# Daaohame/RAHT-3DGS-codec

Measured on AMD Instinct MI355X. Metric: M-Gaussians/s fwd+inv RAHT, 59-ch SH3 3DGS, higher is better.
Workload: dtype f32 (xyz columns: f64); 1 GPU; cfg3: 2999072 Gaussians (3000000 draws/GPU, J=12, 59 channels), fwd RAHT + quantize/reorder + dequantize/un-reorder + inv RAHT (quantization fused into the transform kernels); the 3 xyz columns carried in float64 inside the same launches (raht_fwd_quant_mixed / raht_dequant_inv_mixed): the reference's integers on every column; rows_per_gpu=2999072, channels=59, depth_J=12, engine=tile, quantize=True, parallelism=1 GPU, world=1

## Files before the change

raht-3dgs-codec_amd/csrc/raht_device.h:

```cpp
#pragma once
#include "raht_common.h"

namespace raht {

struct StepTable {
    int n;
    int fast_div;
    float v[MAX_STEP_CH];
};
struct NoSteps { int n; int fast_div; };
struct StepTable64 { int n; double v[MAX_STEP_CH]; };
template <typename T> struct StepsFor;
template <> struct StepsFor<float> { typedef StepTable type; typedef float elem; };
template <> struct StepsFor<double> { typedef StepTable64 type; typedef double elem; };


template <typename E> struct alignas(16) RegChunk { E v[16 / sizeof(E)]; };
template <typename E> struct __attribute__((packed, aligned(sizeof(E)))) MemChunk { E v[16 / sizeof(E)]; };

template <typename E, bool STREAM = false>
__device__ __forceinline__ RegChunk<E> ld_chunk(const E *__restrict__ p)
{
    constexpr int VN = 16 / sizeof(E);
    RegChunk<E> x;
    if constexpr (STREAM) {
#pragma unroll
        for (int i = 0; i < VN; ++i) x.v[i] = __builtin_nontemporal_load(p + i);
    } else {
        const MemChunk<E> t = *(const MemChunk<E> *)p;
#pragma unroll
        for (int i = 0; i < VN; ++i) x.v[i] = t.v[i];
    }
    return x;
}

template <typename E, bool STREAM = false>
__device__ __forceinline__ void st_chunk(E *__restrict__ p, const RegChunk<E> &x)
{
    constexpr int VN = 16 / sizeof(E);
    if constexpr (STREAM) {
#pragma unroll
        for (int i = 0; i < VN; ++i) __builtin_nontemporal_store(x.v[i], p + i);
    } else {
        MemChunk<E> t;
#pragma unroll
        for (int i = 0; i < VN; ++i) t.v[i] = x.v[i];
        *(MemChunk<E> *)p = t;
    }
}

template <int VN> struct __attribute__((packed, aligned(4))) IntPack { int32_t v[VN]; };
// ... 142 lines not shown
```

raht-3dgs-codec_amd/csrc/transform.hip:

```cpp
#include "raht_common.h"
#include "raht_device.h"
#include "tile_engine.h"
#include "tile_host.h"

#include <algorithm>
#include <type_traits>
#include <vector>

namespace raht {

size_t tile_lds_bytes(int R, int elem_size, int Dc, bool ident, bool qm);

template <typename T> struct Vec16;
template <> struct Vec16<float> { typedef float4 type; static constexpr int n = 4; };
template <> struct Vec16<double> { typedef double2 type; static constexpr int n = 2; };

template <typename T>
__global__ void copy_rows_kernel(const T *__restrict__ src, int64_t lds, T *__restrict__ dst, int64_t ldd,
                                 int64_t N, int D)
{
    const int64_t total = N * D;
    for (int64_t e = (int64_t)blockIdx.x * blockDim.x + threadIdx.x; e < total;
         e += (int64_t)gridDim.x * blockDim.x) {
        const int64_t i = e / D;
// ... 642 lines not shown
template <typename T, bool INV, bool IDENT, bool QM, int SLOTS>
__global__ __launch_bounds__(TILE_THREADS, (sizeof(T) == 4 ? 6 : 4)) void tile_kernel_batch(const TileBatch<T> B,
                                                   const typename std::conditional<QM, typename StepsFor<T>::type, NoSteps>::type ST)
{
    int s = 0;
#pragma unroll
    for (int q = 1; q < BATCH_MAX; ++q) s += (q < B.n && blockIdx.x >= B.first_tile[q]) ? 1 : 0;
    const int64_t t = (int64_t)(blockIdx.x - B.first_tile[s]);
    tile_body<T, INV, IDENT, QM, SLOTS>(B.a[s], ST, t, (int64_t)1 << 40, (int)blockIdx.y);
}

constexpr int TOP_THREADS = 1024;
constexpr int TOP_SLOTS = RAHT_TOP_MAX_ROWS / TOP_THREADS;

template <typename T>
struct TopArgs {
    const T *in;  int64_t ld_in;
    T *fin;       int64_t ld_fin;
    T *out;       int64_t ld_out;
    int32_t *Q;   int64_t ldq;
    const uint32_t *rows;
    int io_mapped;
    const uint32_t *e_pos;
    const uint32_t *pj;
    const T *ab;
    const uint32_t *root_rank;
    T *root_buf;
    int n, n_merges, D;
    const uint32_t *lev;
    int nlev, nbig;
    uint32_t small_start;
};

template <typename T, bool INV, bool QM, bool MULTI = false>
__device__ __forceinline__ void top_body(const TopArgs<T> &A, const typename std::conditional<QM, typename StepsFor<T>::type, NoSteps>::type &ST,
                                         const int chunk, const MultiQ *MQ = nullptr)
{
    constexpr bool QM64 = QM && sizeof(T) == 8;
    extern __shared__ __align__(16) unsigned char smem[];
    typedef RegChunk<T> V16;
    constexpr int VN = 16 / sizeof(T);
    V16 *tile = (V16 *)smem;
    __shared__ uint32_t s_lev[2 * 64];
    const int tid = threadIdx.x;
    const int goff = min(chunk * VN, A.D - VN);
    const int n = A.n, nm = A.n_merges;
    if (tid < 2 * A.nlev) s_lev[tid] = A.lev[tid];
    const int n_small = nm - (int)A.small_start;
    uint32_t *s_pj = (uint32_t *)(smem + (size_t)n * 16);
    T *s_ab = (T *)(s_pj + ((n_small + 3) & ~3));
    for (int i = tid; i < n_small; i += TOP_THREADS) {
        s_pj[i] = A.pj[A.small_start + i];
        s_ab[2 * i] = A.ab[2 * (A.small_start + i)];
        s_ab[2 * i + 1] = A.ab[2 * (A.small_start + i) + 1];
    }

    typename StepsFor<T>::elem my_step[VN];
    float my_rcp[VN];
#pragma unroll
    for (int i = 0; i < VN; ++i) { my_step[i] = 1; my_rcp[i] = 1.0f; }
    if constexpr (QM) {
#pragma unroll
        for (int i = 0; i < VN; ++i) {
            my_step[i] = ST.v[ST.n == 1 ? 0 : goff + i];
            if constexpr (!QM64) my_rcp[i] = refined_rcp(my_step[i]);
        }
    }

    uint32_t pj[TOP_SLOTS];
    T ra[TOP_SLOTS], rb[TOP_SLOTS];
#pragma unroll
    for (int k = 0; k < TOP_SLOTS; ++k) {
        const int idx = min(k * TOP_THREADS + tid, max(nm - 1, 0));
        pj[k] = A.pj[idx]; ra[k] = A.ab[2 * idx]; rb[k] = A.ab[2 * idx + 1];
    }
    uint32_t m_dst[TOP_SLOTS], m_rr[TOP_SLOTS];
#pragma unroll
    for (int k = 0; k < TOP_SLOTS; ++k) {
        const int e = min(k * TOP_THREADS + tid, n - 1);
        m_rr[k] = A.root_rank[e];
        m_dst[k] = QM ? A.e_pos[e] : (A.rows ? A.rows[e] : (uint32_t)e);
    }
    {
        typedef typename std::conditional<QM && INV && !QM64, int32_t, T>::type RawT;
        RegChunk<RawT> x[TOP_SLOTS];
#pragma unroll
        for (int k = 0; k < TOP_SLOTS; ++k) {
            const int e = min(k * TOP_THREADS + tid, n - 1);
            if constexpr (QM64 && INV) {
                int32_t q[VN];
                ld_ints<VN>(A.Q + (int64_t)m_dst[k] * A.ldq + goff, q);
#pragma unroll
                for (int i = 0; i < VN; ++i) x[k].v[i] = (T)q[i];
            } else if constexpr (!INV) {
                x[k] = ld_chunk<RawT>((const RawT *)A.in + (int64_t)(A.io_mapped ? m_dst[k] : (uint32_t)e) * A.ld_in + goff);
            } else if constexpr (QM) {
                x[k] = ld_chunk<RawT>((const RawT *)A.Q + (int64_t)m_dst[k] * A.ldq + goff);
            } else {
                const T *src = (A.root_buf && m_rr[k] != 0xffffffffu) ? A.root_buf + (int64_t)m_rr[k] * A.D
                                                                      : A.fin + (int64_t)m_dst[k] * A.ld_fin;
                x[k] = ld_chunk<RawT>((const RawT *)src + goff);
            }
        }
#pragma unroll
        for (int k = 0; k < TOP_SLOTS; ++k) {
            const int e = k * TOP_THREADS + tid;
            if (e < n) {
                V16 v;
#pragma unroll
                for (int i = 0; i < VN; ++i) {
                    v.v[i] = (T)x[k].v[i];
                    if constexpr (QM && INV) v.v[i] = v.v[i] * (T)my_step[i];
                }
                tile[e] = v;
            }
        }
        if constexpr (QM && INV) {
            if (A.root_buf) {
#pragma unroll
                for (int k = 0; k < TOP_SLOTS; ++k) {
                    const int e = k * TOP_THREADS + tid;
                    if (e < n && m_rr[k] != 0xffffffffu) tile[e] = ld_chunk<T>(A.root_buf + (int64_t)m_rr[k] * A.D + goff);
                }
            }
        }
    }
    __syncthreads();

    auto butterfly = [&](uint32_t rec, T a, T b) {
        const uint32_t ip = rec & 0xffffu, ij = rec >> 16;
        const V16 x0 = tile[ip], x1 = tile[ij];
        V16 vlo, vhi;
#pragma unroll
        for (int i = 0; i < VN; ++i) {
            if (!INV) {
                vlo.v[i] = a * x0.v[i] + b * x1.v[i];
                vhi.v[i] = a * x1.v[i] - b * x0.v[i];
            } else {
                vlo.v[i] = a * x0.v[i] - b * x1.v[i];
                vhi.v[i] = b * x0.v[i] + a * x1.v[i];
            }
        }
        tile[ip] = vlo; tile[ij] = vhi;
    };
    auto big_levels = [&]() {
#pragma unroll 1
        for (int q = 0; q < A.nbig; ++q) {
            const int li = INV ? A.nbig - 1 - q : q;
            const uint32_t lo = s_lev[2 * li], hi = s_lev[2 * li + 1];
#pragma unroll
            for (int k = 0; k < TOP_SLOTS; ++k) {
                const uint32_t idx = (uint32_t)(k * TOP_THREADS + tid);
                if ((uint32_t)(k * TOP_THREADS) < hi && (uint32_t)((k + 1) * TOP_THREADS) > lo && idx >= lo && idx < hi)
                    butterfly(pj[k], ra[k], rb[k]);
            }
            __syncthreads();
        }
    };
    auto small_levels = [&]() {
        if (tid < 64) {
#pragma unroll 1
            for (int q = A.nbig; q < A.nlev; ++q) {
                const int li = INV ? A.nlev - 1 - (q - A.nbig) : q;
                const uint32_t lo = s_lev[2 * li], hi = s_lev[2 * li + 1];
                const uint32_t i = lo - A.small_start + (uint32_t)tid;
                if (lo + (uint32_t)tid < hi) butterfly(s_pj[i], s_ab[2 * i], s_ab[2 * i + 1]);
            }
        }
        __syncthreads();
    };
    if (!INV) { big_levels(); small_levels(); }
    else { small_levels(); big_levels(); }

#pragma unroll
    for (int k = 0; k < TOP_SLOTS; ++k) {
        const int e = k * TOP_THREADS + tid;
        if (e >= n) continue;
        const V16 v = tile[e];
        if constexpr (INV) {
            st_chunk<T>(A.out + (int64_t)(A.io_mapped ? m_dst[k] : (uint32_t)e) * A.ld_out + goff, v);
        } else {
            const uint32_t rr = m_rr[k];
            const bool to_buf = A.root_buf && rr != 0xffffffffu;
            if (to_buf) st_chunk<T>(A.root_buf + (int64_t)rr * A.D + goff, v);
            if (QM && to_buf) {
            } else if constexpr (QM) {
                if constexpr (QM64) {
                    int32_t qv[VN];
#pragma unroll
                    for (int i = 0; i < VN; ++i) qv[i] = quantize_one_f64((double)v.v[i], (double)my_step[i]);
                    st_ints<VN>(A.Q + (int64_t)m_dst[k] * A.ldq + goff, qv);
                } else if constexpr (MULTI) {
                    for (int kk = 0; kk < MQ->k; ++kk) {
                        const float sp = MQ->step[kk], rc = refined_rcp(sp);
                        RegChunk<int32_t> qv;
#pragma unroll
                        for (int i = 0; i < VN; ++i) qv.v[i] = quantize_one((float)v.v[i], sp, rc, MQ->fast_div);
                        st_chunk<int32_t>(MQ->Q[kk] + (int64_t)m_dst[k] * A.ldq + goff, qv);
                    }
                } else {
                    RegChunk<int32_t> qv;
#pragma unroll
                    for (int i = 0; i < VN; ++i) qv.v[i] = quantize_one((float)v.v[i], (float)my_step[i], my_rcp[i], ST.fast_div);
                    st_chunk<int32_t>(A.Q + (int64_t)m_dst[k] * A.ldq + goff, qv);
                }
            } else {
                st_chunk<T>(A.fin + (int64_t)m_dst[k] * A.ld_fin + goff, v);
            }
        }
    }
}

template <typename T, bool INV, bool QM>
__global__ __launch_bounds__(TOP_THREADS) void top_kernel(const TopArgs<T> A,
                                                          const typename std::conditional<QM, typename StepsFor<T>::type, NoSteps>::type ST)
{
    top_body<T, INV, QM>(A, ST, (int)blockIdx.x);
}

__global__ __launch_bounds__(TOP_THREADS) void top_kernel_multi(const TopArgs<float> A, const StepTable ST, const MultiQ M)
{
    top_body<float, false, true, true>(A, ST, (int)blockIdx.x, &M);
}

template <typename T>
struct TopBatch { TopArgs<T> a[BATCH_MAX]; };

template <typename T, bool INV, bool QM>
__global__ __launch_bounds__(TOP_THREADS) void top_kernel_batch(const TopBatch<T> B,
                                                                const typename std::conditional<QM, typename StepsFor<T>::type, NoSteps>::type ST)
{
    top_body<T, INV, QM>(B.a[blockIdx.y], ST, (int)blockIdx.x);
}

template <typename T>
__global__ void node_weight_kernel(const int32_t *__restrict__ wl, const int32_t *__restrict__ wr,
                                   const int64_t *__restrict__ wsum, int64_t N, T *__restrict__ w)
{
    const int64_t i = (int64_t)blockIdx.x * blockDim.x + threadIdx.x;
    if (i >= N) return;
    if (i == 0) { w[0] = (T)(wsum ? wsum[N] : N); return; }
    double w0, w1;
    pair_weights(i, wl[i], wr[i], wsum, w0, w1);
    w[i] = (T)(w0 + w1);
}

static int lp_shift_for(int Dc)
{
    int s = 0;
    while ((1 << s) < Dc && s < 6) ++s;
// ... 119 lines not shown
        else if (st.tile_rows < 1 || (int64_t)st.tile_rows * std::max<int64_t>(std::max(A.ld_in, A.ld_out), A.ld_fin) * (int64_t)sizeof(T) >= ((int64_t)1 << 32)) bad = "tile geometry (32-bit row offsets)";
        if (bad) { set_error("tile stage %d (%s): missing %s", k, INV ? "inverse" : "forward", bad); return RAHT_ERR_INVALID; }
    }
    G.nchunks = (unsigned)((D + Dc - 1) / Dc);
    G.lds = tile_lds_bytes(st.tile_rows, (int)sizeof(T), Dc, st.rows == nullptr, QM);
    if (st.tile_rows > TILE_MAX_SLOTS * TILE_THREADS) {
        set_error("tile_rows %d too large for %d threads", st.tile_rows, TILE_THREADS);
        return RAHT_ERR_UNSUPPORTED;
    }
    G.n_tiles = st.n_tiles;
    G.one = st.tile_rows <= TILE_THREADS;
    G.ident = st.rows == nullptr;
    if (sq) {
        if (G.nchunks != 1 || !G.ident || (size_t)(TILE_THREADS / 64) * (size_t)(((D + 3) / 4) * 4) * 8 > G.lds) {
            set_error("raht_dequant_inv_sqdiff: unexpected stage-0 geometry");
            return RAHT_ERR_INVALID;
        }
        if (!A.out) A.ld_out = 0;
        A.ref = io.ref; A.ld_ref = io.ld_ref; A.sq_part = io.sq_part;
    }
    return RAHT_OK;
}

template <typename T, bool INV, bool QM>
static int launch_prepared(const raht_plan *p, int k, const StageLaunch<T> &L, const XformIO<T> &io, bool events, hipStream_t s)
{
    constexpr bool F32Q = QM && std::is_same<T, float>::value;
    const auto st = steps_arg<T, QM>(io);
    auto launch = [&]() -> int {
        if (L.is_top) {
            constexpr int VN = 16 / (int)sizeof(T);
            const dim3 grid((unsigned)((L.P.D + VN - 1) / VN)), block(TOP_THREADS);
            if constexpr (F32Q && !INV) { if (io.multi) return launch_lds<top_kernel_multi>(grid, block, L.G.lds, TOP_LDS_LIMIT, s, L.P, st, *io.multi); }
            return launch_lds<top_kernel<T, INV, QM>>(grid, block, L.G.lds, TOP_LDS_LIMIT, s, L.P, st);
        }
        const TileGeom &G = L.G;
        const dim3 grid((unsigned)G.n_tiles, G.nchunks), block(TILE_THREADS);
        return by_ident_slots(G.ident, G.one, [&](auto ident, auto slots) -> int {
            constexpr bool IDENT = decltype(ident)::value;
            constexpr int SLOTS = decltype(slots)::value;
            if constexpr (F32Q && !INV) { if (io.multi) return launch_lds<tile_kernel_multi<IDENT, SLOTS>>(grid, block, G.lds, TILE_LDS_LIMIT, s, L.A, st, *io.multi); }
            if constexpr (F32Q && INV && IDENT) { if (L.A.sq_part) return launch_lds<tile_kernel_sq<SLOTS>>(grid, block, G.lds, TILE_LDS_LIMIT, s, L.A, st); }
            return launch_lds<tile_kernel<T, INV, IDENT, QM, SLOTS>>(grid, block, G.lds, TILE_LDS_LIMIT, s, L.A, st);
        });
    };
    if (!(events && k == 0 && p->ev_before)) return launch();
    RAHT_HIP_CHECK(hipEventRecord(p->ev_before, s));
    const int rc = launch();
    RAHT_HIP_CHECK(hipEventRecord(p->ev_after, s));
    return rc;
}

template <typename T, bool INV, bool QM>
static int launch_stage(const raht_plan *p, const Schedule &sc, int k, const XformIO<T> &io, int D, int Dc0, hipStream_t s, int dbg = 0)
{
    StageLaunch<T> L;
    RAHT_RET((prepare_stage<T, INV, QM>(p, sc, k, io, D, Dc0, dbg, L)));
    return launch_prepared<T, INV, QM>(p, k, L, io, dbg == 0, s);
}

template <typename T, bool INV, bool QM>
static int launch_tile_batch(int m, const StageLaunch<T> *const *Ls, const XformIO<T> &io, hipStream_t s)
{
    TileBatch<T> B;
    B.n = m;
    uint32_t tot = 0;
    for (int i = 0; i < BATCH_MAX; ++i) {
// ... 490 lines not shown
```

raht-3dgs-codec_amd/csrc/transform_mx.hip:

```cpp
#include "raht_common.h"
#include "raht_device.h"
#include "tile_engine.h"
#include "tile_host.h"

#include <algorithm>
#include <cstdlib>
#include <string>
#include <type_traits>
#include <vector>

namespace raht {

#ifdef RAHT_PHASE_CLOCKS
constexpr int MX_CLK_TILES = 4096, MX_CLK_SLOTS = 12;
__device__ unsigned long long g_phase_clk_mx[MX_CLK_TILES][MX_CLK_SLOTS];
#define MX_STAMP(k) do { if (IDENT && threadIdx.x == 0 && tile_id < MX_CLK_TILES) g_phase_clk_mx[tile_id][k] = __builtin_readcyclecounter(); } while (0)
#else
#define MX_STAMP(k) do { } while (0)
#endif

constexpr int MX_MAX_WIDE = 4;
constexpr int MX_THREADS = 512;
constexpr int MX_TOP_THREADS = 1024;
constexpr int MX_TOP_SLOTS = RAHT_TOP_MAX_ROWS / MX_TOP_THREADS;
// ... 586 lines not shown
    TileArgs<float> a[BATCH_MAX];
    MxPtrs p[BATCH_MAX];
    uint32_t first_tile[BATCH_MAX + 1];
    int n;
};
static_assert(sizeof(TileBatchMX) + sizeof(StepTableMX) <= 4096, "tile_kernel_mx_batch: arguments exceed the 4 KB kernarg segment");

template <bool INV, bool IDENT, int SLOTS>
__global__ __launch_bounds__(MX_THREADS, 6) void tile_kernel_mx_batch(const TileBatchMX B, const StepTableMX ST)
{
    int s = 0;
#pragma unroll
    for (int q = 1; q < BATCH_MAX; ++q) s += (q < B.n && blockIdx.x >= B.first_tile[q]) ? 1 : 0;
    tile_body_mx<INV, IDENT, SLOTS, false>(B.a[s], B.p[s], ST, (int64_t)(blockIdx.x - B.first_tile[s]));
}

struct TopArgsMX {
    const float *in_rows;  int64_t ld_in;
    const float *in_img; const double *in_img_w;
    float *out_rows;       int64_t ld_out;
    float *out_img; double *out_img_w;
    int32_t *Q;            int64_t ldq;
    const uint32_t *e_pos;
    const uint32_t *pj;
    const float *ab32;  const double *ab64;
    int n, n_merges, D, nwide, Fp;
    const uint32_t *lev;
    int nlev, nbig;
    uint32_t small_start;
    const uint32_t *root_rank;
    float *root_f; double *root_w;
};

template <bool WIDE, bool INV, bool ROOTS, bool MULTI = false>
__device__ __forceinline__ void top_body_mx(const TopArgsMX &A, const StepTableMX &ST, const int chunk, const MxMultiQ *MQ = nullptr)
{
    typedef typename std::conditional<WIDE, double, float>::type T;
    constexpr int VN = WIDE ? 2 : 4;
    typedef RegChunk<T> V16;
    extern __shared__ __align__(16) unsigned char smem[];
    V16 *tile = (V16 *)smem;
    __shared__ uint32_t s_lev[2 * 64];
    const int tid = threadIdx.x;
    const int nwide = A.nwide;
    const int goff = WIDE ? 2 * chunk : min(chunk * 4, A.D - 4);
    const int ioff = chunk * 4;
    const int n = A.n, nm = A.n_merges;
    if (tid < 2 * A.nlev) s_lev[tid] = A.lev[tid];
    const T *ab = WIDE ? (const T *)A.ab64 : (const T *)A.ab32;
    const int n_small = nm - (int)A.small_start;
    uint32_t *s_pj = (uint32_t *)(smem + (size_t)n * 16);
    T *s_ab = (T *)(s_pj + ((n_small + 3) & ~3));
    for (int i = tid; i < n_small; i += MX_TOP_THREADS) {
        s_pj[i] = A.pj[A.small_start + i];
        s_ab[2 * i] = ab[2 * (A.small_start + i)];
        s_ab[2 * i + 1] = ab[2 * (A.small_start + i) + 1];
    }
    T my_step[VN];
    float my_rcp[VN];
    bool live[VN];
#pragma unroll
    for (int i = 0; i < VN; ++i) {
        if constexpr (WIDE) { live[i] = goff + i < nwide; my_step[i] = live[i] ? ST.w[goff + i] : 1.0; my_rcp[i] = 1.0f; }
        else { live[i] = !(chunk == 0 && i < nwide); my_step[i] = ST.f.v[ST.f.n == 1 ? 0 : goff + i]; my_rcp[i] = refined_rcp(my_step[i]); }
    }
    uint32_t pj[MX_TOP_SLOTS];
    T ra[MX_TOP_SLOTS], rb[MX_TOP_SLOTS];
#pragma unroll
    for (int k = 0; k < MX_TOP_SLOTS; ++k) {
        const int idx = min(k * MX_TOP_THREADS + tid, max(nm - 1, 0));
        pj[k] = A.pj[idx]; ra[k] = ab[2 * idx]; rb[k] = ab[2 * idx + 1];
    }
    uint32_t m_dst[MX_TOP_SLOTS], m_rr[MX_TOP_SLOTS];
#pragma unroll
    for (int k = 0; k < MX_TOP_SLOTS; ++k) {
        m_dst[k] = A.e_pos[min(k * MX_TOP_THREADS + tid, n - 1)];
        m_rr[k] = ROOTS ? A.root_rank[min(k * MX_TOP_THREADS + tid, n - 1)] : 0xffffffffu;
    }
#pragma unroll
    for (int k = 0; k < MX_TOP_SLOTS; ++k) {
        const int e = k * MX_TOP_THREADS + tid;
        if (e >= n) continue;
        V16 v;
        if constexpr (!INV) {
            if (A.in_img) {
                if constexpr (WIDE) {
#pragma unroll
                    for (int i = 0; i < VN; ++i) v.v[i] = live[i] ? A.in_img_w[(int64_t)e * nwide + goff + i] : 0.0;
                } else {
                    v = *(const V16 *)(A.in_img + (int64_t)e * A.Fp + ioff);
                }
            } else if constexpr (WIDE) {
#pragma unroll
                for (int i = 0; i < VN; ++i) v.v[i] = live[i] ? (double)A.in_rows[(int64_t)e * A.ld_in + goff + i] : 0.0;
            } else {
                v = ld_chunk<float>(A.in_rows + (int64_t)e * A.ld_in + goff);
            }
        } else if (m_rr[k] != 0xffffffffu) {
            if constexpr (WIDE) {
#pragma unroll
                for (int i = 0; i < VN; ++i) v.v[i] = live[i] ? A.root_w[(int64_t)m_rr[k] * nwide + goff + i] : 0.0;
            } else {
                v = ld_chunk<float>(A.root_f + (int64_t)m_rr[k] * A.D + goff);
            }
        } else {
            const int32_t *q = A.Q + (int64_t)m_dst[k] * A.ldq + goff;
            if constexpr (WIDE) {
#pragma unroll
                for (int i = 0; i < VN; ++i) v.v[i] = live[i] ? (double)q[i] * my_step[i] : 0.0;
            } else {
                const RegChunk<int32_t> raw = ld_chunk<int32_t>(q);
#pragma unroll
                for (int i = 0; i < VN; ++i) v.v[i] = (float)raw.v[i] * my_step[i];
            }
        }
        tile[e] = v;
    }
    __syncthreads();

    auto butterfly = [&](uint32_t rec, T a, T b) {
        const uint32_t ip = rec & 0xffffu, ij = rec >> 16;
        const V16 x0 = tile[ip], x1 = tile[ij];
        V16 vlo, vhi;
#pragma unroll
        for (int i = 0; i < VN; ++i) {
            if (!INV) {
                vlo.v[i] = a * x0.v[i] + b * x1.v[i];
                vhi.v[i] = a * x1.v[i] - b * x0.v[i];
            } else {
                vlo.v[i] = a * x0.v[i] - b * x1.v[i];
                vhi.v[i] = b * x0.v[i] + a * x1.v[i];
            }
        }
        tile[ip] = vlo; tile[ij] = vhi;
    };
    auto big_levels = [&]() {
#pragma unroll 1
        for (int q = 0; q < A.nbig; ++q) {
            const int li = INV ? A.nbig - 1 - q : q;
            const uint32_t lo = s_lev[2 * li], hi = s_lev[2 * li + 1];
#pragma unroll
            for (int k = 0; k < MX_TOP_SLOTS; ++k) {
                const uint32_t idx = (uint32_t)(k * MX_TOP_THREADS + tid);
                if ((uint32_t)(k * MX_TOP_THREADS) < hi && (uint32_t)((k + 1) * MX_TOP_THREADS) > lo && idx >= lo && idx < hi)
                    butterfly(pj[k], ra[k], rb[k]);
            }
            __syncthreads();
        }
    };
    auto small_levels = [&]() {
        if (tid < 64) {
#pragma unroll 1
            for (int q = A.nbig; q < A.nlev; ++q) {
                const int li = INV ? A.nlev - 1 - (q - A.nbig) : q;
                const uint32_t lo = s_lev[2 * li], hi = s_lev[2 * li + 1];
                const uint32_t i = lo - A.small_start + (uint32_t)tid;
                if (lo + (uint32_t)tid < hi) butterfly(s_pj[i], s_ab[2 * i], s_ab[2 * i + 1]);
            }
        }
        __syncthreads();
    };
    if (!INV) { big_levels(); small_levels(); }
    else { small_levels(); big_levels(); }

#pragma unroll
    for (int k = 0; k < MX_TOP_SLOTS; ++k) {
        const int e = k * MX_TOP_THREADS + tid;
        if (e >= n) continue;
        const V16 v = tile[e];
        if constexpr (INV) {
            if (A.out_img) {
                if constexpr (WIDE) {
#pragma unroll
                    for (int i = 0; i < VN; ++i) if (live[i]) A.out_img_w[(int64_t)e * nwide + goff + i] = v.v[i];
                } else {
                    *(V16 *)(A.out_img + (int64_t)e * A.Fp + ioff) = v;
                }
            } else if constexpr (WIDE) {
#pragma unroll
                for (int i = 0; i < VN; ++i) if (live[i]) A.out_rows[(int64_t)e * A.ld_out + goff + i] = (float)v.v[i];
            } else if (chunk == 0) {
#pragma unroll
                for (int i = 0; i < VN; ++i) if (live[i]) A.out_rows[(int64_t)e * A.ld_out + goff + i] = v.v[i];
            } else {
                st_chunk<float>(A.out_rows + (int64_t)e * A.ld_out + goff, v);
            }
        } else if (m_rr[k] != 0xffffffffu) {
            if constexpr (WIDE) {
#pragma unroll
                for (int i = 0; i < VN; ++i) if (live[i]) A.root_w[(int64_t)m_rr[k] * nwide + goff + i] = v.v[i];
            } else {
                st_chunk<float>(A.root_f + (int64_t)m_rr[k] * A.D + goff, v);
            }
        } else if constexpr (MULTI) {
            for (int kk = 0; kk < MQ->k; ++kk) {
                int32_t *q = MQ->Q[kk] + (int64_t)m_dst[k] * A.ldq + goff;
                if constexpr (WIDE) {
#pragma unroll
                    for (int i = 0; i < VN; ++i) if (live[i]) q[i] = quantize_one_f64(v.v[i], MQ->step[kk]);
                } else {
                    const float sf = (float)MQ->step[kk], rf = refined_rcp(sf);
                    const int fd = (int)((MQ->fast_div >> kk) & 1u);
                    RegChunk<int32_t> qv;
#pragma unroll
                    for (int i = 0; i < VN; ++i) qv.v[i] = quantize_one(v.v[i], sf, rf, fd);
                    if (chunk == 0) {
#pragma unroll
                        for (int i = 0; i < VN; ++i) if (live[i]) q[i] = qv.v[i];
                    } else {
                        st_chunk<int32_t>(q, qv);
                    }
                }
            }
        } else {
            int32_t *q = A.Q + (int64_t)m_dst[k] * A.ldq + goff;
            if constexpr (WIDE) {
#pragma unroll
                for (int i = 0; i < VN; ++i) if (live[i]) q[i] = quantize_one_f64(v.v[i], my_step[i]);
            } else {
                RegChunk<int32_t> qv;
#pragma unroll
                for (int i = 0; i < VN; ++i) qv.v[i] = quantize_one(v.v[i], my_step[i], my_rcp[i], ST.f.fast_div);
                if (chunk == 0) {
#pragma unroll
                    for (int i = 0; i < VN; ++i) if (live[i]) q[i] = qv.v[i];
                } else {
                    st_chunk<int32_t>(q, qv);
                }
            }
        }
    }
}

template <bool INV>
__global__ __launch_bounds__(MX_TOP_THREADS) void top_kernel_mx(const TopArgsMX A, const StepTableMX ST)
{
    const int NW2 = (A.nwide + 1) >> 1;
    if ((int)blockIdx.x < NW2) top_body_mx<true, INV, false>(A, ST, (int)blockIdx.x);
    else top_body_mx<false, INV, false>(A, ST, (int)blockIdx.x - NW2);
}
template <bool INV>
__global__ __launch_bounds__(MX_TOP_THREADS) void top_kernel_mx_roots(const TopArgsMX A, const StepTableMX ST)
{
    const int NW2 = (A.nwide + 1) >> 1;
    if ((int)blockIdx.x < NW2) top_body_mx<true, INV, true>(A, ST, (int)blockIdx.x);
    else top_body_mx<false, INV, true>(A, ST, (int)blockIdx.x - NW2);
}

struct TopBatchMX { TopArgsMX a[BATCH_MAX]; };
static_assert(sizeof(TopBatchMX) + sizeof(StepTableMX) <= 4096, "top_kernel_mx_batch: arguments exceed the 4 KB kernarg segment");

template <bool INV>
__global__ __launch_bounds__(MX_TOP_THREADS) void top_kernel_mx_batch(const TopBatchMX B, const StepTableMX ST)
{
    const TopArgsMX &A = B.a[blockIdx.y];
    const int NW2 = (A.nwide + 1) >> 1;
    if ((int)blockIdx.x < NW2) top_body_mx<true, INV, false>(A, ST, (int)blockIdx.x);
    else top_body_mx<false, INV, false>(A, ST, (int)blockIdx.x - NW2);
}

__global__ __launch_bounds__(MX_TOP_THREADS) void top_kernel_mx_multi(const TopArgsMX A, const StepTableMX ST, const MxMultiQ M)
{
    const int NW2 = (A.nwide + 1) >> 1;
    if ((int)blockIdx.x < NW2) top_body_mx<true, false, false, true>(A, ST, (int)blockIdx.x, &M);
    else top_body_mx<false, false, false, true>(A, ST, (int)blockIdx.x - NW2, &M);
}

__global__ void mx_cols_to_f64_kernel(const float *__restrict__ C, int64_t ldc, int64_t N, int nwide, double *__restrict__ W)
{
    const int64_t e = (int64_t)blockIdx.x * blockDim.x + threadIdx.x;
    if (e >= N * nwide) return;
    const int64_t i = e / nwide;
// ... 140 lines not shown
        else if (INV && !A.out && !(k == 0 && io.sq_part)) bad = "inverse output";
        else if (k == 0 && io.sq_part && (!INV || !io.ref || A.root_buf || (int64_t)st.tile_rows * io.ld_ref * 4 >= ((int64_t)1 << 31))) bad = "sqdiff reference rows";
        else if (!INV && io.multi && A.root_buf) bad = "multi-step write-back without root buffers";
        else if ((st.rows == nullptr) != (k == 0)) bad = "stage order";
        else if (st.tile_rows < 1 || st.tile_rows > TILE_MAX_SLOTS * MX_THREADS ||
                 (int64_t)st.tile_rows * std::max<int64_t>(io.ldc, g.Dp) * 4 >= ((int64_t)1 << 31)) bad = "tile geometry (32-bit row offsets)";
        if (bad) { set_error("mixed tile stage %d (%s): missing %s", k, INV ? "inverse" : "forward", bad); return RAHT_ERR_INVALID; }
    }
    MxPtrs &P = L.P;
    P.in_w = (!INV && k >= 1) ? ws_k_w : nullptr;
    P.out_w = (INV && k >= 1) ? ws_k_w : nullptr;
    P.wsn_w = ws_n_w;
    P.root_w = A.last_stage ? p->root_buf_w : nullptr;
    P.prog = st.prog; P.prog_stride = st.prog_stride; P.prog_ab = st.prog_ab; P.prog_compact = st.prog_compact ? 1 : 0;
    if (!P.prog) { set_error("mixed tile stage %d: missing tile programs", k); return RAHT_ERR_INVALID; }
    L.lds = tile_lds_bytes_mx(st.tile_rows, g.Dp / 4, g.nwide);
    L.n_tiles = (unsigned)st.n_tiles;
    if (INV && k == 0 && io.sq_part) {
        A.out = io.C_out; A.ld_out = io.C_out ? io.ldc : 0;
        A.ref = io.ref; A.ld_ref = io.ld_ref; A.sq_part = io.sq_part;
    }
    return RAHT_OK;
}

template <bool INV>
static int launch_prepared_mx(const raht_plan *p, int k, const MxIO &io, const MxStageLaunch &L, const MxGeom &g,
                              const StepTableMX &stp, hipStream_t s)
{
    auto launch = [&]() -> int {
        if (L.is_top) {
            const dim3 grid((unsigned)g.NCp), block(MX_TOP_THREADS);
            if constexpr (!INV) { if (io.multi) return launch_lds<top_kernel_mx_multi>(grid, block, L.lds, TOP_LDS_LIMIT, s, L.T, stp, *io.multi); }
            if (L.T.root_f) return launch_lds<top_kernel_mx_roots<INV>>(grid, block, L.lds, TOP_LDS_LIMIT, s, L.T, stp);
            return launch_lds<top_kernel_mx<INV>>(grid, block, L.lds, TOP_LDS_LIMIT, s, L.T, stp);
        }
        if constexpr (!INV) { if (io.multi) return launch_tile_mx<false, false, MX_MULTI>(k == 0, L.A, L.P, stp, io.multi, L.n_tiles, L.lds, s); }
        if constexpr (INV) { if (k == 0 && io.sq_part) return launch_tile_mx<true, false, MX_SQ>(true, L.A, L.P, stp, nullptr, L.n_tiles, L.lds, s); }
        return L.A.root_buf ? launch_tile_mx<INV, true, MX_PLAIN>(k == 0, L.A, L.P, stp, nullptr, L.n_tiles, L.lds, s)
                            : launch_tile_mx<INV, false, MX_PLAIN>(k == 0, L.A, L.P, stp, nullptr, L.n_tiles, L.lds, s);
    };
    if (!(k == 0 && p->ev_before)) return launch();
    RAHT_HIP_CHECK(hipEventRecord(p->ev_before, s));
    const int rc = launch();
    RAHT_HIP_CHECK(hipEventRecord(p->ev_after, s));
    return rc;
}

template <bool INV>
static int launch_stage_mx(const raht_plan *p, const Schedule &sc, int k, const MxIO &io, int D, const MxGeom &g,
                           const StepTableMX &stp, hipStream_t s)
{
    MxStageLaunch L;
    RAHT_RET((prepare_stage_mx<INV>(p, sc, k, io, D, g, L)));
    return launch_prepared_mx<INV>(p, k, io, L, g, stp, s);
}

static int mx_check_args(const raht_plan *p, const void *a, const void *b, int D, int64_t lda, int64_t ldb, const double *steps,
                         int n_steps, int n_wide, const char *what)
{
    if (!p || !a || !b || D < 1 || lda < D || ldb < D) { set_error("%s: bad argument", what); return RAHT_ERR_INVALID; }
    RAHT_RET(check_plan_device(p, what));
    if (n_wide < 1 || n_wide > MX_MAX_WIDE || n_wide > D) { set_error("%s: n_wide must be 1..%d (and <= D)", what, MX_MAX_WIDE); return RAHT_ERR_INVALID; }
    RAHT_RET(check_quant_steps(what, steps, n_steps, D, true));
    if (p->row_map) { set_error("%s: not available for row-mapped plans", what); return RAHT_ERR_UNSUPPORTED; }
    if ((p->root_buf == nullptr) != (p->root_buf_w == nullptr)) {
        set_error("%s: set both root buffers (raht_plan_set_root_buffer and raht_plan_set_root_buffer_wide) or neither", what);
        return RAHT_ERR_UNSUPPORTED;
// ... 433 lines not shown
```

Baseline: 5001 M-Gaussians/s.

## Restructure top-level RAHT kernel loads for latency hiding and specialize slot count

The top-of-tree kernels now issue index, row-chunk and root loads up front, batched between scheduling barriers, and stage the small-level merge records into LDS through registers after the main loads are issued. Slot count becomes a template parameter, so small top levels launch with 1 or 2 slots and skip unused loads and butterflies. The store loop exits per wave rather than per lane. The aim is to cut serialized global-memory latency in these small, latency-bound top kernels, at the cost of more registers and extra kernel instantiations.

```diff
diff --git a/raht-3dgs-codec_amd/csrc/raht_device.h b/raht-3dgs-codec_amd/csrc/raht_device.h
--- a/raht-3dgs-codec_amd/csrc/raht_device.h
+++ b/raht-3dgs-codec_amd/csrc/raht_device.h
@@ -17,6 +17,7 @@
 
 template <typename E> struct alignas(16) RegChunk { E v[16 / sizeof(E)]; };
 template <typename E> struct __attribute__((packed, aligned(sizeof(E)))) MemChunk { E v[16 / sizeof(E)]; };
+struct __attribute__((packed, aligned(4), may_alias)) RawChunk { uint32_t v[4]; };
 
 template <typename E, bool STREAM = false>
 __device__ __forceinline__ RegChunk<E> ld_chunk(const E *__restrict__ p)
diff --git a/raht-3dgs-codec_amd/csrc/transform.hip b/raht-3dgs-codec_amd/csrc/transform.hip
--- a/raht-3dgs-codec_amd/csrc/transform.hip
+++ b/raht-3dgs-codec_amd/csrc/transform.hip
@@ -698,7 +698,7 @@
     uint32_t small_start;
 };
 
-template <typename T, bool INV, bool QM, bool MULTI = false>
+template <typename T, bool INV, bool QM, bool MULTI = false, int SLOTS = TOP_SLOTS>
 __device__ __forceinline__ void top_body(const TopArgs<T> &A, const typename std::conditional<QM, typename StepsFor<T>::type, NoSteps>::type &ST,
                                          const int chunk, const MultiQ *MQ = nullptr)
 {
@@ -711,15 +711,36 @@
     const int tid = threadIdx.x;
     const int goff = min(chunk * VN, A.D - VN);
     const int n = A.n, nm = A.n_merges;
-    if (tid < 2 * A.nlev) s_lev[tid] = A.lev[tid];
+    uint32_t m_dst[SLOTS], m_rr[SLOTS];
+#pragma unroll
+    for (int k = 0; k < SLOTS; ++k) {
+        const int e = min(k * TOP_THREADS + tid, n - 1);
+        m_rr[k] = A.root_rank[e];
+        m_dst[k] = QM ? A.e_pos[e] : (A.rows ? A.rows[e] : (uint32_t)e);
+    }
+    const uint32_t lev_word = A.lev[min(tid, 2 * 64 - 1)];
     const int n_small = nm - (int)A.small_start;
     uint32_t *s_pj = (uint32_t *)(smem + (size_t)n * 16);
     T *s_ab = (T *)(s_pj + ((n_small + 3) & ~3));
-    for (int i = tid; i < n_small; i += TOP_THREADS) {
-        s_pj[i] = A.pj[A.small_start + i];
-        s_ab[2 * i] = A.ab[2 * (A.small_start + i)];
-        s_ab[2 * i + 1] = A.ab[2 * (A.small_start + i) + 1];
-    }
+    constexpr int STAGE = 2;
+    const int nm_last = max(nm - 1, 0);
+    uint32_t g_pj[STAGE];
+    T g_a[STAGE], g_b[STAGE];
+    auto stage_load = [&](int base) {
+#pragma unroll
+        for (int q = 0; q < STAGE; ++q) {
+            const int idx = min((int)A.small_start + base + q * TOP_THREADS + tid, nm_last);
+            g_pj[q] = A.pj[idx]; g_a[q] = A.ab[2 * idx]; g_b[q] = A.ab[2 * idx + 1];
+        }
+    };
+    auto stage_store = [&](int base) {
+#pragma unroll
+        for (int q = 0; q < STAGE; ++q) {
+            const int i = base + q * TOP_THREADS + tid;
+            if (i < n_small) { s_pj[i] = g_pj[q]; s_ab[2 * i] = g_a[q]; s_ab[2 * i + 1] = g_b[q]; }
+        }
+    };
+    stage_load(0);
 
     typename StepsFor<T>::elem my_step[VN];
     float my_rcp[VN];
@@ -733,43 +754,65 @@
         }
     }
 
-    uint32_t pj[TOP_SLOTS];
-    T ra[TOP_SLOTS], rb[TOP_SLOTS];
-#pragma unroll
-    for (int k = 0; k < TOP_SLOTS; ++k) {
+    uint32_t pj[SLOTS];
+    T ra[SLOTS], rb[SLOTS];
+#pragma unroll
+    for (int k = 0; k < SLOTS; ++k) {
         const int idx = min(k * TOP_THREADS + tid, max(nm - 1, 0));
         pj[k] = A.pj[idx]; ra[k] = A.ab[2 * idx]; rb[k] = A.ab[2 * idx + 1];
     }
-    uint32_t m_dst[TOP_SLOTS], m_rr[TOP_SLOTS];
-#pragma unroll
-    for (int k = 0; k < TOP_SLOTS; ++k) {
-        const int e = min(k * TOP_THREADS + tid, n - 1);
-        m_rr[k] = A.root_rank[e];
-        m_dst[k] = QM ? A.e_pos[e] : (A.rows ? A.rows[e] : (uint32_t)e);
-    }
     {
         typedef typename std::conditional<QM && INV && !QM64, int32_t, T>::type RawT;
-        RegChunk<RawT> x[TOP_SLOTS];
-#pragma unroll
-        for (int k = 0; k < TOP_SLOTS; ++k) {
-            const int e = min(k * TOP_THREADS + tid, n - 1);
+        RegChunk<RawT> x[SLOTS];
+        const void *src[SLOTS];
+        uint32_t in_row[SLOTS];
+#pragma unroll
+        for (int k = 0; k < SLOTS; ++k) in_row[k] = (uint32_t)min(k * TOP_THREADS + tid, n - 1);
+        if constexpr (!INV) {
+            if (A.io_mapped) {
+                asm volatile("" ::: "memory");
+#pragma unroll
+                for (int k = 0; k < SLOTS; ++k) in_row[k] = m_dst[k];
+            }
+        }
+#pragma unroll
+        for (int k = 0; k < SLOTS; ++k) {
+            if constexpr (!INV) {
+                src[k] = A.in + (int64_t)in_row[k] * A.ld_in + goff;
+            } else if constexpr (QM) {
+                int64_t off = (int64_t)m_dst[k] * A.ldq;
+                if constexpr (!QM64) {
+                    if (A.root_buf && m_rr[k] != 0xffffffffu) off = ((const int32_t *)A.root_buf - A.Q) + (int64_t)m_rr[k] * A.D;
+                }
+                src[k] = A.Q + goff + off;
+            } else {
+                src[k] = (A.root_buf && m_rr[k] != 0xffffffffu) ? A.root_buf + (int64_t)m_rr[k] * A.D + goff
+                                                                : A.fin + (int64_t)m_dst[k] * A.ld_fin + goff;
+            }
+        }
+        __builtin_amdgcn_sched_barrier(0);
+#pragma unroll
+        for (int k = 0; k < SLOTS; ++k) {
             if constexpr (QM64 && INV) {
                 int32_t q[VN];
-                ld_ints<VN>(A.Q + (int64_t)m_dst[k] * A.ldq + goff, q);
+                ld_ints<VN>((const int32_t *)src[k], q);
 #pragma unroll
                 for (int i = 0; i < VN; ++i) x[k].v[i] = (T)q[i];
-            } else if constexpr (!INV) {
-                x[k] = ld_chunk<RawT>((const RawT *)A.in + (int64_t)(A.io_mapped ? m_dst[k] : (uint32_t)e) * A.ld_in + goff);
-            } else if constexpr (QM) {
-                x[k] = ld_chunk<RawT>((const RawT *)A.Q + (int64_t)m_dst[k] * A.ldq + goff);
+            } else if constexpr (QM && INV) {
+                const RawChunk t = *(const RawChunk *)src[k];
+#pragma unroll
+                for (int i = 0; i < VN; ++i) x[k].v[i] = (RawT)t.v[i];
             } else {
-                const T *src = (A.root_buf && m_rr[k] != 0xffffffffu) ? A.root_buf + (int64_t)m_rr[k] * A.D
-                                                                      : A.fin + (int64_t)m_dst[k] * A.ld_fin;
-                x[k] = ld_chunk<RawT>((const RawT *)src + goff);
-            }
-        }
-#pragma unroll
-        for (int k = 0; k < TOP_SLOTS; ++k) {
+                x[k] = ld_chunk<RawT>((const RawT *)src[k]);
+            }
+        }
+        __builtin_amdgcn_sched_barrier(0);
+        s_lev[min(tid, 2 * 64 - 1)] = lev_word;
+        stage_store(0);
+#pragma unroll 1
+        for (int base = STAGE * TOP_THREADS; base < n_small; base += STAGE * TOP_THREADS) { stage_load(base); stage_store(base); }
+#pragma unroll
+        for (int k = 0; k < SLOTS; ++k) {
             const int e = k * TOP_THREADS + tid;
             if (e < n) {
                 V16 v;
@@ -777,16 +820,23 @@
                 for (int i = 0; i < VN; ++i) {
                     v.v[i] = (T)x[k].v[i];
                     if constexpr (QM && INV) v.v[i] = v.v[i] * (T)my_step[i];
+                    if constexpr (QM && INV && !QM64) {
+                        if (A.root_buf && m_rr[k] != 0xffffffffu) v.v[i] = __int_as_float(x[k].v[i]);
+                    }
                 }
                 tile[e] = v;
             }
         }
-        if constexpr (QM && INV) {
+        if constexpr (QM64 && INV) {
             if (A.root_buf) {
-#pragma unroll
-                for (int k = 0; k < TOP_SLOTS; ++k) {
+                V16 r[SLOTS];
+#pragma unroll
+                for (int k = 0; k < SLOTS; ++k)
+                    r[k] = ld_chunk<T>(A.root_buf + (int64_t)(m_rr[k] != 0xffffffffu ? m_rr[k] : 0u) * A.D + goff);
+#pragma unroll
+                for (int k = 0; k < SLOTS; ++k) {
                     const int e = k * TOP_THREADS + tid;
-                    if (e < n && m_rr[k] != 0xffffffffu) tile[e] = ld_chunk<T>(A.root_buf + (int64_t)m_rr[k] * A.D + goff);
+                    if (e < n && m_rr[k] != 0xffffffffu) tile[e] = r[k];
                 }
             }
         }
@@ -815,7 +865,7 @@
             const int li = INV ? A.nbig - 1 - q : q;
             const uint32_t lo = s_lev[2 * li], hi = s_lev[2 * li + 1];
 #pragma unroll
-            for (int k = 0; k < TOP_SLOTS; ++k) {
+            for (int k = 0; k < SLOTS; ++k) {
                 const uint32_t idx = (uint32_t)(k * TOP_THREADS + tid);
                 if ((uint32_t)(k * TOP_THREADS) < hi && (uint32_t)((k + 1) * TOP_THREADS) > lo && idx >= lo && idx < hi)
                     butterfly(pj[k], ra[k], rb[k]);
@@ -838,10 +888,11 @@
     if (!INV) { big_levels(); small_levels(); }
     else { small_levels(); big_levels(); }
 
-#pragma unroll
-    for (int k = 0; k < TOP_SLOTS; ++k) {
-        const int e = k * TOP_THREADS + tid;
-        if (e >= n) continue;
+    const int wave_first = __builtin_amdgcn_readfirstlane(tid) & ~63;
+#pragma unroll
+    for (int k = 0; k < SLOTS; ++k) {
+        if (k * TOP_THREADS + wave_first >= n) break;
+        const int e = min(k * TOP_THREADS + tid, n - 1);
         const V16 v = tile[e];
         if constexpr (INV) {
             st_chunk<T>(A.out + (int64_t)(A.io_mapped ? m_dst[k] : (uint32_t)e) * A.ld_out + goff, v);
@@ -877,11 +928,11 @@
     }
 }
 
-template <typename T, bool INV, bool QM>
+template <typename T, bool INV, bool QM, int SLOTS>
 __global__ __launch_bounds__(TOP_THREADS) void top_kernel(const TopArgs<T> A,
                                                           const typename std::conditional<QM, typename StepsFor<T>::type, NoSteps>::type ST)
 {
-    top_body<T, INV, QM>(A, ST, (int)blockIdx.x);
+    top_body<T, INV, QM, false, SLOTS>(A, ST, (int)blockIdx.x);
 }
 
 __global__ __launch_bounds__(TOP_THREADS) void top_kernel_multi(const TopArgs<float> A, const StepTable ST, const MultiQ M)
@@ -1067,7 +1118,9 @@
             constexpr int VN = 16 / (int)sizeof(T);
             const dim3 grid((unsigned)((L.P.D + VN - 1) / VN)), block(TOP_THREADS);
             if constexpr (F32Q && !INV) { if (io.multi) return launch_lds<top_kernel_multi>(grid, block, L.G.lds, TOP_LDS_LIMIT, s, L.P, st, *io.multi); }
-            return launch_lds<top_kernel<T, INV, QM>>(grid, block, L.G.lds, TOP_LDS_LIMIT, s, L.P, st);
+            if (L.P.n <= TOP_THREADS) return launch_lds<top_kernel<T, INV, QM, 1>>(grid, block, L.G.lds, TOP_LDS_LIMIT, s, L.P, st);
+            if (L.P.n <= 2 * TOP_THREADS) return launch_lds<top_kernel<T, INV, QM, 2>>(grid, block, L.G.lds, TOP_LDS_LIMIT, s, L.P, st);
+            return launch_lds<top_kernel<T, INV, QM, TOP_SLOTS>>(grid, block, L.G.lds, TOP_LDS_LIMIT, s, L.P, st);
         }
         const TileGeom &G = L.G;
         const dim3 grid((unsigned)G.n_tiles, G.nchunks), block(TILE_THREADS);
diff --git a/raht-3dgs-codec_amd/csrc/transform_mx.hip b/raht-3dgs-codec_amd/csrc/transform_mx.hip
--- a/raht-3dgs-codec_amd/csrc/transform_mx.hip
+++ b/raht-3dgs-codec_amd/csrc/transform_mx.hip
@@ -642,7 +642,7 @@
     float *root_f; double *root_w;
 };
 
-template <bool WIDE, bool INV, bool ROOTS, bool MULTI = false>
+template <bool WIDE, bool INV, bool ROOTS, bool MULTI = false, int SLOTS = MX_TOP_SLOTS>
 __device__ __forceinline__ void top_body_mx(const TopArgsMX &A, const StepTableMX &ST, const int chunk, const MxMultiQ *MQ = nullptr)
 {
     typedef typename std::conditional<WIDE, double, float>::type T;
@@ -656,16 +656,36 @@
     const int goff = WIDE ? 2 * chunk : min(chunk * 4, A.D - 4);
     const int ioff = chunk * 4;
     const int n = A.n, nm = A.n_merges;
-    if (tid < 2 * A.nlev) s_lev[tid] = A.lev[tid];
     const T *ab = WIDE ? (const T *)A.ab64 : (const T *)A.ab32;
     const int n_small = nm - (int)A.small_start;
     uint32_t *s_pj = (uint32_t *)(smem + (size_t)n * 16);
     T *s_ab = (T *)(s_pj + ((n_small + 3) & ~3));
-    for (int i = tid; i < n_small; i += MX_TOP_THREADS) {
-        s_pj[i] = A.pj[A.small_start + i];
-        s_ab[2 * i] = ab[2 * (A.small_start + i)];
-        s_ab[2 * i + 1] = ab[2 * (A.small_start + i) + 1];
-    }
+    uint32_t m_dst[SLOTS], m_rr[SLOTS];
+#pragma unroll
+    for (int k = 0; k < SLOTS; ++k) {
+        m_dst[k] = A.e_pos[min(k * MX_TOP_THREADS + tid, n - 1)];
+        m_rr[k] = ROOTS ? A.root_rank[min(k * MX_TOP_THREADS + tid, n - 1)] : 0xffffffffu;
+    }
+    const uint32_t lev_word = A.lev[min(tid, 2 * 64 - 1)];
+    constexpr int STAGE = ROOTS ? 1 : 2;
+    const int nm_last = max(nm - 1, 0);
+    uint32_t g_pj[STAGE];
+    T g_a[STAGE], g_b[STAGE];
+    auto stage_load = [&](int base) {
+#pragma unroll
+        for (int q = 0; q < STAGE; ++q) {
+            const int idx = min((int)A.small_start + base + q * MX_TOP_THREADS + tid, nm_last);
+            g_pj[q] = A.pj[idx]; g_a[q] = ab[2 * idx]; g_b[q] = ab[2 * idx + 1];
+        }
+    };
+    auto stage_store = [&](int base) {
+#pragma unroll
+        for (int q = 0; q < STAGE; ++q) {
+            const int i = base + q * MX_TOP_THREADS + tid;
+            if (i < n_small) { s_pj[i] = g_pj[q]; s_ab[2 * i] = g_a[q]; s_ab[2 * i + 1] = g_b[q]; }
+        }
+    };
+    stage_load(0);
     T my_step[VN];
     float my_rcp[VN];
     bool live[VN];
@@ -674,58 +694,111 @@
         if constexpr (WIDE) { live[i] = goff + i < nwide; my_step[i] = live[i] ? ST.w[goff + i] : 1.0; my_rcp[i] = 1.0f; }
         else { live[i] = !(chunk == 0 && i < nwide); my_step[i] = ST.f.v[ST.f.n == 1 ? 0 : goff + i]; my_rcp[i] = refined_rcp(my_step[i]); }
     }
-    uint32_t pj[MX_TOP_SLOTS];
-    T ra[MX_TOP_SLOTS], rb[MX_TOP_SLOTS];
-#pragma unroll
-    for (int k = 0; k < MX_TOP_SLOTS; ++k) {
-        const int idx = min(k * MX_TOP_THREADS + tid, max(nm - 1, 0));
-        pj[k] = A.pj[idx]; ra[k] = ab[2 * idx]; rb[k] = ab[2 * idx + 1];
-    }
-    uint32_t m_dst[MX_TOP_SLOTS], m_rr[MX_TOP_SLOTS];
-#pragma unroll
-    for (int k = 0; k < MX_TOP_SLOTS; ++k) {
-        m_dst[k] = A.e_pos[min(k * MX_TOP_THREADS + tid, n - 1)];
-        m_rr[k] = ROOTS ? A.root_rank[min(k * MX_TOP_THREADS + tid, n - 1)] : 0xffffffffu;
-    }
-#pragma unroll
-    for (int k = 0; k < MX_TOP_SLOTS; ++k) {
+    uint32_t pj[SLOTS];
+    T ra[SLOTS], rb[SLOTS];
+    auto load_records = [&]() {
+#pragma unroll
+        for (int k = 0; k < SLOTS; ++k) {
+            const int idx = min(k * MX_TOP_THREADS + tid, nm_last);
+            pj[k] = A.pj[idx]; ra[k] = ab[2 * idx]; rb[k] = ab[2 * idx + 1];
+        }
+    };
+    constexpr bool RECORDS_LATE = WIDE && INV && ROOTS;
+    if constexpr (!RECORDS_LATE) load_records();
+    V16 x[SLOTS];
+    int wch[VN];
+#pragma unroll
+    for (int i = 0; i < VN; ++i) wch[i] = WIDE ? min(goff + i, nwide - 1) : 0;
+    if constexpr (!INV) {
+        if (A.in_img) {
+#pragma unroll
+            for (int k = 0; k < SLOTS; ++k) {
+                const int e = min(k * MX_TOP_THREADS + tid, n - 1);
+                if constexpr (WIDE) {
+#pragma unroll
+                    for (int i = 0; i < VN; ++i) x[k].v[i] = A.in_img_w[(int64_t)e * nwide + wch[i]];
+                } else {
+                    x[k] = *(const V16 *)(A.in_img + (int64_t)e * A.Fp + ioff);
+                }
+            }
+        } else {
+#pragma unroll
+            for (int k = 0; k < SLOTS; ++k) {
+                const int e = min(k * MX_TOP_THREADS + tid, n - 1);
+                if constexpr (WIDE) {
+#pragma unroll
+                    for (int i = 0; i < VN; ++i) x[k].v[i] = (double)A.in_rows[(int64_t)e * A.ld_in + wch[i]];
+                } else {
+                    x[k] = ld_chunk<float>(A.in_rows + (int64_t)e * A.ld_in + goff);
+                }
+            }
+        }
+    } else if constexpr (WIDE) {
+        int32_t qi[SLOTS][VN];
+        double rw[SLOTS][VN];
+        const int32_t *qp[SLOTS];
+        const double *rp[SLOTS];
+#pragma unroll
+        for (int k = 0; k < SLOTS; ++k) {
+            qp[k] = A.Q + (int64_t)m_dst[k] * A.ldq;
+            rp[k] = A.root_w + (int64_t)(m_rr[k] != 0xffffffffu ? m_rr[k] : 0u) * nwide;
+        }
+        __builtin_amdgcn_sched_barrier(0);
+#pragma unroll
+        for (int k = 0; k < SLOTS; ++k) {
+#pragma unroll
+            for (int i = 0; i < VN; ++i) {
+                qi[k][i] = qp[k][wch[i]];
+                rw[k][i] = ROOTS ? rp[k][wch[i]] : 0.0;
+            }
+        }
+        __builtin_amdgcn_sched_barrier(0);
+#pragma unroll
+        for (int k = 0; k < SLOTS; ++k)
+#pragma unroll
+            for (int i = 0; i < VN; ++i) {
+                const double dq = (double)qi[k][i] * my_step[i];
+                x[k].v[i] = (ROOTS && m_rr[k] != 0xffffffffu) ? rw[k][i] : dq;
+            }
+    } else {
+        RawChunk raw[SLOTS];
+        const int32_t *base = A.Q + goff;
+        const int64_t root_base = ROOTS ? (const int32_t *)A.root_f - A.Q : 0;
+        int64_t off[SLOTS];
+#pragma unroll
+        for (int k = 0; k < SLOTS; ++k) {
+            off[k] = (int64_t)m_dst[k] * A.ldq;
+            if (ROOTS && m_rr[k] != 0xffffffffu) off[k] = root_base + (int64_t)m_rr[k] * A.D;
+        }
+        __builtin_amdgcn_sched_barrier(0);
+#pragma unroll
+        for (int k = 0; k < SLOTS; ++k) raw[k] = *(const RawChunk *)(base + off[k]);
+        __builtin_amdgcn_sched_barrier(0);
+#pragma unroll
+        for (int k = 0; k < SLOTS; ++k)
+#pragma unroll
+            for (int i = 0; i < VN; ++i) {
+                const float dq = (float)(int32_t)raw[k].v[i] * my_step[i];
+                x[k].v[i] = (ROOTS && m_rr[k] != 0xffffffffu) ? __uint_as_float(raw[k].v[i]) : dq;
+            }
+    }
+    s_lev[min(tid, 2 * 64 - 1)] = lev_word;
+    stage_store(0);
+#pragma unroll 1
+    for (int base = STAGE * MX_TOP_THREADS; base < n_small; base += STAGE * MX_TOP_THREADS) { stage_load(base); stage_store(base); }
+#pragma unroll
+    for (int k = 0; k < SLOTS; ++k) {
         const int e = k * MX_TOP_THREADS + tid;
-        if (e >= n) continue;
-        V16 v;
-        if constexpr (!INV) {
-            if (A.in_img) {
-                if constexpr (WIDE) {
-#pragma unroll
-                    for (int i = 0; i < VN; ++i) v.v[i] = live[i] ? A.in_img_w[(int64_t)e * nwide + goff + i] : 0.0;
-                } else {
-                    v = *(const V16 *)(A.in_img + (int64_t)e * A.Fp + ioff);
-                }
-            } else if constexpr (WIDE) {
-#pragma unroll
-                for (int i = 0; i < VN; ++i) v.v[i] = live[i] ? (double)A.in_rows[(int64_t)e * A.ld_in + goff + i] : 0.0;
-            } else {
-                v = ld_chunk<float>(A.in_rows + (int64_t)e * A.ld_in + goff);
-            }
-        } else if (m_rr[k] != 0xffffffffu) {
+        if (e < n) {
+            V16 v = x[k];
             if constexpr (WIDE) {
 #pragma unroll
-                for (int i = 0; i < VN; ++i) v.v[i] = live[i] ? A.root_w[(int64_t)m_rr[k] * nwide + goff + i] : 0.0;
-            } else {
-                v = ld_chunk<float>(A.root_f + (int64_t)m_rr[k] * A.D + goff);
-            }
-        } else {
-            const int32_t *q = A.Q + (int64_t)m_dst[k] * A.ldq + goff;
-            if constexpr (WIDE) {
-#pragma unroll
-                for (int i = 0; i < VN; ++i) v.v[i] = live[i] ? (double)q[i] * my_step[i] : 0.0;
-            } else {
-                const RegChunk<int32_t> raw = ld_chunk<int32_t>(q);
-#pragma unroll
-                for (int i = 0; i < VN; ++i) v.v[i] = (float)raw.v[i] * my_step[i];
-            }
-        }
-        tile[e] = v;
-    }
+                for (int i = 0; i < VN; ++i) if (!live[i]) v.v[i] = 0.0;
+            }
+            tile[e] = v;
+        }
+    }
+    if constexpr (RECORDS_LATE) load_records();
     __syncthreads();
 
     auto butterfly = [&](uint32_t rec, T a, T b) {
@@ -750,7 +823,7 @@
             const int li = INV ? A.nbig - 1 - q : q;
             const uint32_t lo = s_lev[2 * li], hi = s_lev[2 * li + 1];
 #pragma unroll
-            for (int k = 0; k < MX_TOP_SLOTS; ++k) {
+            for (int k = 0; k < SLOTS; ++k) {
                 const uint32_t idx = (uint32_t)(k * MX_TOP_THREADS + tid);
                 if ((uint32_t)(k * MX_TOP_THREADS) < hi && (uint32_t)((k + 1) * MX_TOP_THREADS) > lo && idx >= lo && idx < hi)
                     butterfly(pj[k], ra[k], rb[k]);
@@ -773,10 +846,11 @@
     if (!INV) { big_levels(); small_levels(); }
     else { small_levels(); big_levels(); }
 
-#pragma unroll
-    for (int k = 0; k < MX_TOP_SLOTS; ++k) {
-        const int e = k * MX_TOP_THREADS + tid;
-        if (e >= n) continue;
+    const int wave_first = __builtin_amdgcn_readfirstlane(tid) & ~63;
+#pragma unroll
+    for (int k = 0; k < SLOTS; ++k) {
+        if (k * MX_TOP_THREADS + wave_first >= n) break;
+        const int e = min(k * MX_TOP_THREADS + tid, n - 1);
         const V16 v = tile[e];
         if constexpr (INV) {
             if (A.out_img) {
@@ -842,12 +916,12 @@
     }
 }
 
-template <bool INV>
+template <bool INV, int SLOTS>
 __global__ __launch_bounds__(MX_TOP_THREADS) void top_kernel_mx(const TopArgsMX A, const StepTableMX ST)
 {
     const int NW2 = (A.nwide + 1) >> 1;
-    if ((int)blockIdx.x < NW2) top_body_mx<true, INV, false>(A, ST, (int)blockIdx.x);
-    else top_body_mx<false, INV, false>(A, ST, (int)blockIdx.x - NW2);
+    if ((int)blockIdx.x < NW2) top_body_mx<true, INV, false, false, SLOTS>(A, ST, (int)blockIdx.x);
+    else top_body_mx<false, INV, false, false, SLOTS>(A, ST, (int)blockIdx.x - NW2);
 }
 template <bool INV>
 __global__ __launch_bounds__(MX_TOP_THREADS) void top_kernel_mx_roots(const TopArgsMX A, const StepTableMX ST)
@@ -1054,7 +1128,9 @@
             const dim3 grid((unsigned)g.NCp), block(MX_TOP_THREADS);
             if constexpr (!INV) { if (io.multi) return launch_lds<top_kernel_mx_multi>(grid, block, L.lds, TOP_LDS_LIMIT, s, L.T, stp, *io.multi); }
             if (L.T.root_f) return launch_lds<top_kernel_mx_roots<INV>>(grid, block, L.lds, TOP_LDS_LIMIT, s, L.T, stp);
-            return launch_lds<top_kernel_mx<INV>>(grid, block, L.lds, TOP_LDS_LIMIT, s, L.T, stp);
+            if (L.T.n <= MX_TOP_THREADS) return launch_lds<top_kernel_mx<INV, 1>>(grid, block, L.lds, TOP_LDS_LIMIT, s, L.T, stp);
+            if (L.T.n <= 2 * MX_TOP_THREADS) return launch_lds<top_kernel_mx<INV, 2>>(grid, block, L.lds, TOP_LDS_LIMIT, s, L.T, stp);
+            return launch_lds<top_kernel_mx<INV, MX_TOP_SLOTS>>(grid, block, L.lds, TOP_LDS_LIMIT, s, L.T, stp);
         }
         if constexpr (!INV) { if (io.multi) return launch_tile_mx<false, false, MX_MULTI>(k == 0, L.A, L.P, stp, io.multi, L.n_tiles, L.lds, s); }
         if constexpr (INV) { if (k == 0 && io.sq_part) return launch_tile_mx<true, false, MX_SQ>(true, L.A, L.P, stp, nullptr, L.n_tiles, L.lds, s); }
```

Measured after the change: 4975 M-Gaussians/s. No clear change (-0.5%).
